# Runki2018/litehandnet

Hardware: AMD Instinct MI355X
Metric: images/sec fwd+bwd @256x256 bs64 litehandnet (higher is better)
Workload: dtype f32; 1 GPU; litehandnet variant B (MSRB hourglass litehourglass.py) C=128, 256x256x3 -> 21x64x64, per-GPU batch 64, train-mode BN, fwd + TopdownHeatmapLoss + bwd + fused Adam; global_batch=64, parallelism=dp1

## Files before the change

### include/lhn.h

```cpp
#ifndef LHN_H
#define LHN_H
#include <stdint.h>
#ifdef __cplusplus
extern "C" {
#endif

#define LHN_VERSION 3
#define LHN_STAT_REPLICAS 32

typedef struct lhn_view {
  float*       data;
  const float* table;
  const float* gate;
  int32_t N, H, W;
  int32_t cstride;
  int32_t coff;
  int32_t C;
  const void* pend;
} lhn_view;

typedef struct lhn_gradview {
  const float* dz;
  const float* dpool;
  const float* coef;
// ... 278 lines not shown
  double*      sums[2];
  int32_t      lo[2], C[2];
  int32_t      n;
} lhn_bn_slices;
int lhn_gate_bwd_reduce2(const lhn_view* y, const float* dz, float* dgate , float* tsum,
                         const lhn_bn_slices* slices, void* stream);
int lhn_gate_bwd_reduce3(const lhn_view* y, const float* dz, float* dgate, float* tsum, const lhn_bn_slices* slices, int prezeroed,
                         void* stream);
typedef struct lhn_gatesum {
  float*               dgate;
  const lhn_bn_slices* slices;
} lhn_gatesum;
int lhn_conv_pw_bwd5(const lhn_view* x, const float* w, const lhn_view* y, const lhn_gradview* gy, float* dx, int dx_accumulate,
                     float* dw, float* dbias, int stride, const float* dy_nchw, int nrep, int64_t rep_stride,
                     const lhn_pw_opts* opts, const lhn_bnsum* bns, const lhn_bnbwdsrc* fin, const lhn_gatesum* gs, void* stream);
int lhn_avgpool_fwd3(const lhn_view* x, float* out , int OH, int OW, float* pstat ,
                     const lhn_bn_slices* slices, void* stream);
int lhn_ca_mlp_bwd2(const float* pooled, const float* w3, const float* gamma, const float* w1, const float* w2,
                    const float* dropmask, const float* save, const float* dgate, float* dpool, int cstride, int coff, int H,
                    int W, float* dw3, float* dgamma, float* dbeta, float* dw1, float* db1, float* dw2, float* db2, int N, int C,
                    int stage, double* gsum, double count_scale, float pgrad_scale, const float* tsum, const float* pstat,
                    const lhn_bn_slices* slices, void* stream);
int lhn_avgpool_fwd4(const lhn_view* x, float* out, int OH, int OW, float* pstat, const lhn_bn_slices* slices,
                     const lhn_view* copy_src, void* stream);
int lhn_ca_mlp_bwd(const float* pooled, const float* w3, const float* gamma, const float* w1, const float* w2,
                   const float* dropmask, const float* save, const float* dgate, float* dpool ,
                   int cstride, int coff, int H, int W, float* dw3, float* dgamma, float* dbeta, float* dw1,
                   float* db1, float* dw2, float* db2, int N, int C, int stage, double* gsum, double count_scale,
                   float pgrad_scale, void* stream);

// ... 14 lines not shown
  int32_t out_buf, out_coff, out_C;
  int32_t p[12];
  int64_t ws[12];
  int32_t i[8];
  float   f[8];
} lhn_op;

typedef struct lhn_buf {
  int64_t data_off, table_off, gate_off, grad_off, dpool_off, coef_off;
  int32_t N, H, W, C;
} lhn_buf;

void* lhn_plan_create(const lhn_buf* bufs, int nbufs, const lhn_op* fwd, int nfwd, const lhn_op* bwd, int nbwd);
void  lhn_plan_destroy(void* plan);
int   lhn_plan_head_gate_fold(void* plan);
#define LHN_RUN_TABLES_CURRENT 2
#define LHN_RUN_GRAPH 4
int   lhn_plan_run(void* plan, int phase, void* workspace, void* const* params, void* const* grads,
                   void* const* io, int training, int grad_replicas, int64_t grad_rep_stride, void* stream);

#ifdef __cplusplus
}
#endif
#endif
```

### litehandnet_amd/_lib.py

```python
import ctypes as C
import os

import torch

_HERE = os.path.dirname(os.path.abspath(__file__))
LIB_PATH = os.path.join(_HERE, "liblhn.so")
_lib = None


class LhnError(RuntimeError):
    pass


class View(C.Structure):
    _fields_ = [("data", C.c_void_p), ("table", C.c_void_p), ("gate", C.c_void_p),
                ("N", C.c_int32), ("H", C.c_int32), ("W", C.c_int32),
                ("cstride", C.c_int32), ("coff", C.c_int32), ("C", C.c_int32), ("pend", C.c_void_p)]


class GradView(C.Structure):
    _fields_ = [("dz", C.c_void_p), ("dpool", C.c_void_p), ("coef", C.c_void_p)]


class Op(C.Structure):
# ... 5 lines not shown

class Buf(C.Structure):
    _fields_ = [("data_off", C.c_int64), ("table_off", C.c_int64), ("gate_off", C.c_int64),
                ("grad_off", C.c_int64), ("dpool_off", C.c_int64), ("coef_off", C.c_int64),
                ("N", C.c_int32), ("H", C.c_int32), ("W", C.c_int32), ("C", C.c_int32)]


SYMBOLS = [
    "lhn_version", "lhn_deterministic", "lhn_last_error", "lhn_device_ok",
    "lhn_heatmap_encode", "lhn_heatmap_argmax", "lhn_heatmap_refine", "lhn_transform_preds",
    "lhn_heatmap_decode", "lhn_heatmap_decode_dark", "lhn_heatmap_decode_dark_udp", "lhn_heatmap_nms", "lhn_heatmap_topk", "lhn_pck_accuracy",
    "lhn_eval_state_bytes", "lhn_eval_accumulate", "lhn_eval_finalize",
    "lhn_loss_balanced_mse_fwd", "lhn_loss_balanced_mse_bwd", "lhn_affine_warp_normalize", "lhn_affine_warp_normalize2", "lhn_random_flip", "lhn_hsv_jitter", "lhn_simdr_encode", "lhn_simdr_loss_fwd", "lhn_simdr_loss_bwd",
    "lhn_conv_pw_fwd", "lhn_conv_pw_fwd2", "lhn_conv_pw_bwd2", "lhn_conv_dw_fwd", "lhn_conv_dw_fwd2", "lhn_conv_dw_fwd3", "lhn_conv_pw_dw3_fwd", "lhn_conv_dw3_pw_fwd", "lhn_msrb_round_scratch_bytes", "lhn_msrb_round_fwd", "lhn_bottleneck_fwd", "lhn_stem_tail_fwd", "lhn_conv_stem_fwd", "lhn_conv_kxk_fwd", "lhn_conv_kxk_fwd_bf16x3",
    "lhn_bn_finalize", "lhn_table_fill", "lhn_table_bias", "lhn_fold_bn", "lhn_ew_fwd", "lhn_ew_fwd2", "lhn_ew_fwd3", "lhn_ew_mul_bwd", "lhn_bilinear_bwd", "lhn_shuffle2_fwd", "lhn_shuffle2_bwd", "lhn_bn_finalize2", "lhn_bn_bwd_finalize2", "lhn_maxpool2_fwd", "lhn_avgpool_fwd", "lhn_avgpool_fwd2", "lhn_avgpool_bwd2", "lhn_se_mlp_fwd2", "lhn_se_mlp_bwd2", "lhn_ca_mlp_fwd", "lhn_att_mlp_fwd", "lhn_att_mlp_bwd", "lhn_se_mlp_fwd", "lhn_se_mlp_bwd",
    "lhn_bn_bwd_reduce", "lhn_bn_bwd_finalize", "lhn_conv_pw_bwd", "lhn_conv_dw_bwd", "lhn_conv_dw_bwd2", "lhn_conv_dw_bwd3", "lhn_conv_dw_bwd4", "lhn_conv_pw_bwd4", "lhn_conv_pw_bwd5", "lhn_plan_head_gate_fold", "lhn_conv_stem_bwd",
    "lhn_conv_kxk_bwd", "lhn_ew_bwd", "lhn_ew_bwd2", "lhn_maxpool2_bwd", "lhn_maxpool2_bwd2", "lhn_maxpool2_bwd3", "lhn_ew_bwd3", "lhn_ew_bwd_multi", "lhn_avgpool_bwd3", "lhn_conv_pw_bwd3", "lhn_avgpool_bwd", "lhn_gate_bwd_reduce", "lhn_gate_bwd_reduce2", "lhn_gate_bwd_reduce3", "lhn_adam_step", "lhn_avgpool_fwd3", "lhn_avgpool_fwd4", "lhn_ca_mlp_bwd2",
    "lhn_ca_mlp_bwd", "lhn_reduce_replicas", "lhn_fold_stat_replicas", "lhn_plan_create", "lhn_plan_destroy", "lhn_plan_run", "lhn_plan_run_range",
    "lhn_cbam_layout", "lhn_cbam_fwd", "lhn_cbam_bwd",
]


def lib():
    global _lib
    if _lib is None:
        if not os.path.exists(LIB_PATH):
            raise LhnError(f"{LIB_PATH} is missing: run `python -m litehandnet_amd.build` "
                           "(hipcc --offload-arch=gfx950); there is no CPU fallback")
        _lib = C.CDLL(LIB_PATH)
        _lib.lhn_last_error.restype = C.c_char_p
        _lib.lhn_plan_create.restype = C.c_void_p
# ... 56 lines not shown
```

### litehandnet_amd/csrc/k_conv_dw.hip

```cpp
#include <stdlib.h>
#include "lhn_common.h"

template <int K>
__global__ void __launch_bounds__(256) k_dw_fwd(lhn_view x, const float* __restrict__ w, lhn_view y,
                                                double* __restrict__ stats, int stride, int pad, int dil, lhn_bnfin fin,
                                                int ) {
  extern __shared__ __attribute__((aligned(16))) float smem[];
  const int C = x.C, C4 = C >> 2;
  constexpr int KK = K * K;
  float* Ws = smem;
  f4* red = reinterpret_cast<f4*>(smem + KK * C);
  const int tid = threadIdx.x;
  const int c4 = tid % C4, pl = tid / C4, PL = 256 / C4;
  const int cin = x.coff + 4 * c4, cout = y.coff + 4 * c4;
  const Xf4 xf = lhn_load_xf(x, cin);
  for (int i = tid; i < KK * C; i += 256) {
    const int c = i / KK, t = i - c * KK;
    Ws[t * C + c] = w ? w[i] : 1.f;
  }
  __syncthreads();
  f4 wt[KK];
#pragma unroll
  for (int t = 0; t < KK; ++t) wt[t] = *reinterpret_cast<const f4*>(Ws + t * C + 4 * c4);
  const int rows = y.N * y.H;
// ... 1178 lines not shown
  if (stats) {
    const int C = x.C;
    double* st = stats + (size_t)((bid / cgroups) % LHN_STAT_REPLICAS) * 2 * C + cg * 32;
    lhn_block_stat_atomics_d(sd, qd, 8, reinterpret_cast<double*>(red), st, st + C, cvalid);
    if (fin.counter && lhn_last_block(fin.counter)) lhn_bn_finalize_block_par(fin, stats, reinterpret_cast<double*>(red));
  }
}

struct DwBnSum {
  double* sums;
  const float* save;
  int C, coff;
  const float* add[2];
};

template <int K, int DIL, bool BNS = false>
__global__ void __launch_bounds__(256) k_dwk_bwd_lds(lhn_view x, const float* __restrict__ w, lhn_view y, lhn_gradview gy,
                                                     float* __restrict__ dx, int dx_acc, float* __restrict__ dw, int tiles_h,
                                                     int tiles_w, int cgroups, int nrep, int64_t rep_stride, int ps, DwBnSum bs, int xchunk) {
  constexpr int TH = 8, TW = 16, KK = K * K;
  const int bid = xchunk ? (int)(blockIdx.x & 7) * xchunk + (int)(blockIdx.x >> 3) : (int)blockIdx.x;
  constexpr bool REGACC = (K == 3);
  using T = DwTile<K, DIL, TH, TW>;
  extern __shared__ __attribute__((aligned(16))) float smem[];
  f4* tdy = reinterpret_cast<f4*>(smem);
  f4* tx = tdy + T::PIX * 8;
  f4* red = tx + T::PIX * 8;
  f4* wl = red + 256;
  f4* dws = wl + KK * 8;
  f4* traw = dws + KK * 8;
  f4* tmi = traw + TH * TW * 8;
  const int tid = threadIdx.x, c4 = tid & 7, pl = tid >> 3;
  const int colw = pl & 15, rpar = pl >> 4;
  const int ntile = y.N * ps * ps * tiles_h * tiles_w * cgroups;
  const int cg = bid % cgroups;
  const int cvalid = min(8, (x.C - cg * 32) >> 2);
  const bool cok = c4 < cvalid;
  const int c4e = cok ? c4 : 0;
  const int cx = x.coff + cg * 32 + 4 * c4e, cy = y.coff + cg * 32 + 4 * c4e;
  const Xf4 xxf = lhn_load_xf(x, cx), yxf = lhn_load_xf(y, cy);
  const Gr4 ygr = lhn_load_coef(gy, y.cstride, cy);
  for (int i = tid; i < KK * 8; i += 256) {
    const int k = i >> 3, cc = cg * 32 + 4 * min(i & 7, cvalid - 1);
    wl[i] = (f4){w[(cc + 0) * KK + k], w[(cc + 1) * KK + k], w[(cc + 2) * KK + k], w[(cc + 3) * KK + k]};
    if (!REGACC) dws[i] = (f4){0.f, 0.f, 0.f, 0.f};
  }
  f4 accw[REGACC ? KK : 1];
#pragma unroll
  for (int k = 0; k < (REGACC ? KK : 1); ++k) accw[k] = (f4){0.f, 0.f, 0.f, 0.f};
  f4 sdu = (f4){0.f, 0.f, 0.f, 0.f}, sdux = sdu;
  if (BNS && tid < 16) {
    const int kind = tid >> 3, cc = tid & 7;
    tmi[tid] = *reinterpret_cast<const f4*>(bs.save + kind * bs.C + bs.coff + cg * 32 + 4 * cc);
  }
  for (int t = bid; t < ntile; t += gridDim.x) {
    int r = t / cgroups;
// ... 395 lines not shown
static void launch_dwk_fwd(const lhn_view* x, const float* w, const lhn_view* y, double* stats, lhn_bnfin fin, hipStream_t s, int ps = 1,
                           const DwExtra* exp = nullptr) {
  DwExtra ex;
  if (exp) ex = *exp; else { ex.n = 0; ex.sum_out = nullptr; }
  constexpr int TH = 8, TW = 32, P = DIL * (K - 1) / 2;
  const int cg = (x->C + 31) / 32;
  const int sh = (y->H + ps - 1) / ps, sw = (y->W + ps - 1) / ps;
  const int th = (sh + TH - 1) / TH, tw = (sw + TW - 1) / TW, ntile = y->N * ps * ps * th * tw * cg;
  const size_t lds = (size_t)((TH + 2 * P) * (TW + 2 * P) * 8 + 512 + K * K * 8) * 16;
  const int per_cu = lds > 80 * 1024 ? 1 : (lds > 52 * 1024 ? 2 : 3);
  static LhnKernelCfg cfg;
  (void)lhn_kernel_cfg(cfg, &k_dwk_fwd_lds<K, DIL, NS>, lds, 4, nullptr);
  const int grid = dw3_grid(ntile, cg, per_cu * 2);
  hipLaunchKernelGGL((k_dwk_fwd_lds<K, DIL, NS>), dim3(grid), dim3(256), lds, s, *x, w, *y, stats, th, tw, cg, fin, ps, ex, dw3_xchunk(grid, cg));
}
template <int K, int DIL, bool BNS = false>
static void launch_dwk_bwd(const lhn_view* x, const float* w, const lhn_view* y, const lhn_gradview* gy, float* dx, int dx_acc,
                           float* dw, int nrep, int64_t rep_stride, hipStream_t s, int ps = 1, const DwBnSum* bsp = nullptr) {
  constexpr int TH = 8, TW = 16, P = DIL * (K - 1) / 2;
  DwBnSum bs;
  if (bsp) bs = *bsp; else { bs.sums = nullptr; bs.save = nullptr; bs.C = bs.coff = 0; bs.add[0] = bs.add[1] = nullptr; }
  const int cg = (x->C + 31) / 32;
  const int sh = (x->H + ps - 1) / ps, sw = (x->W + ps - 1) / ps;
  const int th = (sh + TH - 1) / TH, tw = (sw + TW - 1) / TW, ntile = x->N * ps * ps * th * tw * cg;
  const size_t lds = (size_t)((TH + 2 * P) * (TW + 2 * P) * 16 + 256 + 2 * K * K * 8 + (BNS ? TH * TW * 8 + 16 : 0)) * 16;
  static LhnKernelCfg cfg;
  (void)lhn_kernel_cfg(cfg, &k_dwk_bwd_lds<K, DIL, BNS>, lds, 4, nullptr);
  const int grid = dw3_grid(ntile, cg, 4);
  hipLaunchKernelGGL((k_dwk_bwd_lds<K, DIL, BNS>), dim3(grid), dim3(256), lds, s, *x, w, *y, *gy, dx, dx_acc, dw, th, tw,
                     cg, nrep, rep_stride, ps, bs, dw3_xchunk(grid, cg));
}
template <int DIL, bool BNS = false>
static void launch_dw3_bwd_rows(const lhn_view* x, const float* w, const lhn_view* y, const lhn_gradview* gy, float* dx, int dx_acc,
                                float* dw, int nrep, int64_t rep_stride, hipStream_t s, int ps = 1, const DwBnSum* bsp = nullptr,
                                const lhn_bnbwdsrc* fsp = nullptr) {
  constexpr int P = DIL, R = 2 * P + 2, WW = 32 + 2 * P;
  DwBnSum bs;
  if (bsp) bs = *bsp; else { bs.sums = nullptr; bs.save = nullptr; bs.C = bs.coff = 0; bs.add[0] = bs.add[1] = nullptr; }
  lhn_bnbwdsrc fs;
  if (fsp) fs = *fsp; else memset(&fs, 0, sizeof(fs));
  static_assert(R * WW * 8 * 16 >= 2 * LHN_FIN_THREADS * 8, "dy ring holds the replica fold's partials");
  const int cg = (x->C + 31) / 32;
  const int sh = (x->H + ps - 1) / ps, sw = (x->W + ps - 1) / ps;
  const int nstrips = (sw + 31) / 32;
  const size_t lds = (size_t)(2 * R * WW * 8 + 2 * 9 * 8 + 16 + (BNS ? R * 32 * 8 : 0)) * 16;
// ... 6 lines not shown
  const int CH = (sh + nch - 1) / nch;
  nch = (sh + CH - 1) / CH;
  const int ntile = base * nch;
  const int grid = dw3_grid(ntile, cg, per_cu);
  hipLaunchKernelGGL((k_dw3_bwd_rows<DIL, BNS>), dim3(grid), dim3(256), lds, s, *x, w, *y, *gy, dx, dx_acc, dw, nstrips, nch, CH, cg,
                     nrep, rep_stride, ps, bs, fs);
}
static bool lhn_dw_bwd_v1() {
  static int v = -1;
  if (v < 0) {
    const char* e = getenv("LHN_DW_BWD_V1");
    v = (e && e[0] == '1') ? 1 : 0;
  }
  return v == 1;
}


struct DwS2 {
  static constexpr int TH = 4, TW = 16, XH = 2 * TH + 1, XW = 2 * TW + 1, XPIX = XH * XW, DH = TH + 1, DW = TW + 1, DPIX = DH * DW;
};

__global__ void __launch_bounds__(256) k_dws2_fwd_lds(lhn_view x, const float* __restrict__ w, lhn_view y, double* __restrict__ stats,
                                                      int tiles_h, int tiles_w, int cgroups, lhn_bnfin fin) {
  using T = DwS2;
  extern __shared__ __attribute__((aligned(16))) float smem[];
  f4* tx = reinterpret_cast<f4*>(smem);
  f4* red = tx + T::XPIX * 8;
  f4* wl = red + 512;
  const int tid = threadIdx.x, c4 = tid & 7, pl = tid >> 3;
  const int ntile = y.N * tiles_h * tiles_w * cgroups;
// ... 237 lines not shown
    else if (k == 3 && dil == 2 && y->W >= 16) launch_dwk_fwd<3, 1, 2>(x, w, y, stats, fin, s, 2, ex);
    else return 0;
    return 1;
  }
  if (k == 3 && dil == 1) launch_dwk_fwd<3, 1>(x, w, y, stats, fin, s, 1, ex);
  else if (k == 3 && dil == 2 && y->W >= 16) launch_dwk_fwd<3, 1>(x, w, y, stats, fin, s, 2, ex);
  else if (k == 3 && dil == 2) launch_dwk_fwd<3, 2>(x, w, y, stats, fin, s, 1, ex);
  else if (k == 7 && dil == 1) launch_dwk_fwd<7, 1>(x, w, y, stats, fin, s, 1, ex);
  else return 0;
  return 1;
}
int lhn_dwk_bwd_lds(const lhn_view* x, const float* w, const lhn_view* y, const lhn_gradview* gy, float* dx, int dx_acc,
                    float* dw, int k, int dil, int nrep, int64_t rep_stride, hipStream_t s, const DwBnSum* bs,
                    const lhn_bnbwdsrc* fs) {
  if (fs && (lhn_dw_bwd_v1() || k != 3)) return 0;
  if (bs && bs->sums) {
    if (!(k == 3 && dil == 1 && dx && !dx_acc)) return 0;
    if (lhn_dw_bwd_v1()) launch_dwk_bwd<3, 1, true>(x, w, y, gy, dx, dx_acc, dw, nrep, rep_stride, s, 1, bs);
    else launch_dw3_bwd_rows<1, true>(x, w, y, gy, dx, dx_acc, dw, nrep, rep_stride, s, 1, bs, fs);
    return 1;
  }
  const bool v1 = lhn_dw_bwd_v1();
  if (k == 3 && dil == 1) {
    if (v1) launch_dwk_bwd<3, 1>(x, w, y, gy, dx, dx_acc, dw, nrep, rep_stride, s, 1, bs);
    else launch_dw3_bwd_rows<1>(x, w, y, gy, dx, dx_acc, dw, nrep, rep_stride, s, 1, bs, fs);
  } else if (k == 3 && dil == 2 && x->W >= 16) {
    if (v1) launch_dwk_bwd<3, 1>(x, w, y, gy, dx, dx_acc, dw, nrep, rep_stride, s, 2, bs);
    else launch_dw3_bwd_rows<1>(x, w, y, gy, dx, dx_acc, dw, nrep, rep_stride, s, 2, bs, fs);
  } else if (k == 3 && dil == 2) {
    if (v1) launch_dwk_bwd<3, 2>(x, w, y, gy, dx, dx_acc, dw, nrep, rep_stride, s, 1, bs);
    else launch_dw3_bwd_rows<2>(x, w, y, gy, dx, dx_acc, dw, nrep, rep_stride, s, 1, bs, fs);
  } else if (k == 7 && dil == 1) launch_dwk_bwd<7, 1>(x, w, y, gy, dx, dx_acc, dw, nrep, rep_stride, s, 1, bs);
  else return 0;
  return 1;
}

static int dw_fwd_extra(const lhn_view* x, const float* w, const lhn_view* y, double* stats, int k, int stride, int pad, int dil,
                        lhn_bnfin fin, const lhn_view* extra, const float* coef, const lhn_view* so, hipStream_t s) {
  if (!(stride == 1 && pad == dil * (k - 1) / 2 && x->C % 4 == 0 && y->W >= 8)) return 0;
// ... 47 lines not shown
```

### litehandnet_amd/csrc/k_conv_pw.hip

```cpp
#include <stdlib.h>
#include "lhn_common.h"

struct PwGeom {
  int wstride, kvalid, wrows, yacc, statC;
  int64_t nchw_bstride;
};

template <int CIN>
__device__ __forceinline__ void pw_stage_w(float* Ws, int LDA, const float* __restrict__ w, int rows_pad, const PwGeom& g) {
  constexpr int C4 = CIN / 4;
  const bool vec = (g.wstride % 4 == 0) && (g.kvalid % 4 == 0) && ((reinterpret_cast<uintptr_t>(w) & 15) == 0);
  for (int i = threadIdx.x; i < rows_pad * C4; i += 256) {
    const int co = i / C4, k4 = i % C4;
    f4 v = (f4){0.f, 0.f, 0.f, 0.f};
    if (co < g.wrows) {
      const float* r = w + (int64_t)co * g.wstride + k4 * 4;
      if (vec) {
        if (4 * k4 < g.kvalid) v = *reinterpret_cast<const f4*>(r);
      } else {
        if (4 * k4 + 0 < g.kvalid) v.x = r[0];
        if (4 * k4 + 1 < g.kvalid) v.y = r[1];
        if (4 * k4 + 2 < g.kvalid) v.z = r[2];
        if (4 * k4 + 3 < g.kvalid) v.w = r[3];
      }
// ... 1242 lines not shown
                                int64_t rep_stride, const lhn_pw_opts* opts, void* stream) {
  return lhn_conv_pw_bwd3(x, w, y, gy, dx, dx_accumulate, dw, dbias, stride, dy_nchw, nrep, rep_stride, opts, nullptr, stream);
}
extern "C" int lhn_conv_pw_bwd3(const lhn_view* x, const float* w, const lhn_view* y, const lhn_gradview* gy, float* dx,
                                int dx_accumulate, float* dw, float* dbias, int stride, const float* dy_nchw, int nrep,
                                int64_t rep_stride, const lhn_pw_opts* opts, const lhn_bnsum* bns, void* stream) {
  return lhn_conv_pw_bwd4(x, w, y, gy, dx, dx_accumulate, dw, dbias, stride, dy_nchw, nrep, rep_stride, opts, bns, nullptr, stream);
}
extern "C" int lhn_conv_pw_bwd4(const lhn_view* x, const float* w, const lhn_view* y, const lhn_gradview* gy, float* dx,
                                int dx_accumulate, float* dw, float* dbias, int stride, const float* dy_nchw, int nrep,
                                int64_t rep_stride, const lhn_pw_opts* opts, const lhn_bnsum* bns, const lhn_bnbwdsrc* fin, void* stream) {
  return lhn_conv_pw_bwd5(x, w, y, gy, dx, dx_accumulate, dw, dbias, stride, dy_nchw, nrep, rep_stride, opts, bns, fin, nullptr, stream);
}
static int pw_bwd_run(const lhn_view* x, const float* w, const lhn_view* y, const lhn_gradview* gy, float* dx, int dx_accumulate, float* dw,
                      float* dbias, int stride, const float* dy_nchw, int nrep, int64_t rep_stride, const lhn_pw_opts* opts,
                      const lhn_bnsum* bns, const lhn_bnbwdsrc* fin, const lhn_gatesum* gs, bool* gs_done, void* stream);
extern "C" int lhn_conv_pw_bwd5(const lhn_view* x, const float* w, const lhn_view* y, const lhn_gradview* gy, float* dx,
                                int dx_accumulate, float* dw, float* dbias, int stride, const float* dy_nchw, int nrep,
                                int64_t rep_stride, const lhn_pw_opts* opts, const lhn_bnsum* bns, const lhn_bnbwdsrc* fin,
                                const lhn_gatesum* gs, void* stream) {
  if (gs && !gs->dgate) gs = nullptr;
  if (gs) LHN_CHECK_ARG(lhn_view_ok(x) && dx && !dx_accumulate && stride == 1 && (!gs->slices || (gs->slices->n >= 0 && gs->slices->n <= 2)),
                        "lhn_conv_pw_bwd5: gate sums need a stored dx (no accumulate), stride 1 and 0..2 BatchNorm slices");
  bool gs_done = false;
  const int rc = pw_bwd_run(x, w, y, gy, dx, dx_accumulate, dw, dbias, stride, dy_nchw, nrep, rep_stride, opts, bns, fin, gs, &gs_done, stream);
  if (rc || !gs || gs_done) return rc;
  lhn_view xv = *x;
  xv.gate = nullptr;
  return lhn_gate_bwd_reduce3(&xv, dx, gs->dgate, gs->dgate + (size_t)x->N * x->cstride, gs->slices, 1, stream);
}
static int pw_bwd_run(const lhn_view* x, const float* w, const lhn_view* y, const lhn_gradview* gy, float* dx, int dx_accumulate, float* dw,
                      float* dbias, int stride, const float* dy_nchw, int nrep, int64_t rep_stride, const lhn_pw_opts* opts,
                      const lhn_bnsum* bns, const lhn_bnbwdsrc* fin, const lhn_gatesum* gs, bool* gs_done, void* stream) {
  if (nrep < 1) nrep = 1;
  if (fin && !fin->sums) fin = nullptr;
  lhn_bnsum bs;
  memset(&bs, 0, sizeof(bs));
  if (bns && bns->sums) {
    LHN_CHECK_ARG(x && y && bns->save && dx && stride == 1 && x->C <= 128 && y->C <= 128 && x->C * y->C < 64 * 128 && !x->gate && x->table &&
                      bns->coff >= 0 && bns->coff + x->C <= bns->C,
                  "lhn_conv_pw_bwd3: BatchNorm sums ride in the fused kernel only (stride 1, Cin * Cout < 8192, ungated input inside the producer's channels)");
    bs = *bns;
  }
  LHN_CHECK_ARG(lhn_view_ok(x) && w && y && gy && dw && lhn_no_pend(x) && lhn_no_pend(y), "lhn_conv_pw_bwd: bad view / null pointer");
  LHN_CHECK_ARG(stride == 1 || stride == 2, "lhn_conv_pw_bwd: stride %d", stride);
  LHN_CHECK_ARG(stride == 1 || !dx || dx_accumulate, "lhn_conv_pw_bwd: stride-2 dgrad only accumulates into a zeroed gradient");
  if (!dy_nchw) LHN_CHECK_ARG(lhn_view_ok(y) && gy->dz, "lhn_conv_pw_bwd: bad output view / missing dz");
  const int Cout = y->C, Cin = x->C, HoWo = y->H * y->W;
// ... 15 lines not shown
    *gs_done = gs != nullptr;
    return 0;
  }
  if (fin) {
    LHN_CHECK_ARG(!dy_nchw && gy->coef && fin->save_mean_invstd && fin->count > 0 && fin->stat_channels >= Cout,
                  "lhn_conv_pw_bwd4: finalize source needs gy->coef, saved statistics and stat_channels >= Cout");
    if (!wr_wide && !wr_narrow) {
      const int rc = lhn_bn_bwd_finalize2(fin->sums, fin->gamma, fin->save_mean_invstd, const_cast<float*>(gy->coef), y->cstride, y->coff,
                                          Cout, fin->stat_channels, fin->count, fin->dgamma, fin->dbeta, fin->pgrad_scale, stream);
      if (rc) return rc;
      fin = nullptr;
    }
  }
  if (wr_wide) {
    int rc = -1;
    if (Cin == 128 && Cout == 128) rc = launch_pw_bwd_wr<128, 128, 32, 1>(x, w, y, gy, dx, dx_accumulate, dw, dbias, nrep, rep_stride, s, bs, fin);
    else if (Cin == 64 && Cout == 128) rc = launch_pw_bwd_wr<64, 128, 64, 1>(x, w, y, gy, dx, dx_accumulate, dw, dbias, nrep, rep_stride, s, bs, fin);
    else if (Cin == 128 && Cout == 64) rc = launch_pw_bwd_wr<128, 64, 64, 2>(x, w, y, gy, dx, dx_accumulate, dw, dbias, nrep, rep_stride, s, bs, fin);
    if (rc == 0) {
      LHN_CHECK_LAUNCH("lhn_conv_pw_bwd");
      return 0;
    }
    if (rc > 0) return rc;
  }
  if (wr_narrow) {
    int rc;
    if (Cin == 64) rc = bs.sums ? launch_pw_bwd_wr<64, 64, 64, 2, false, true>(x, w, y, gy, dx, dx_accumulate, dw, dbias, nrep, rep_stride, s, bs, fin)
                                : launch_pw_bwd_wr<64, 64, 64, 2, false, false>(x, w, y, gy, dx, dx_accumulate, dw, dbias, nrep, rep_stride, s, bs, fin);
    else rc = bs.sums ? launch_pw_bwd_wr<32, 32, 128, 2, false, true>(x, w, y, gy, dx, dx_accumulate, dw, dbias, nrep, rep_stride, s, bs, fin)
                      : launch_pw_bwd_wr<32, 32, 128, 2, false, false, 3>(x, w, y, gy, dx, dx_accumulate, dw, dbias, nrep, rep_stride, s, bs, fin);
    if (rc) return rc;
    LHN_CHECK_LAUNCH("lhn_conv_pw_bwd");
    return 0;
// ... 52 lines not shown
```

### litehandnet_amd/csrc/lhn_plan.cpp

```cpp
#include <stdint.h>
#include <stdlib.h>
#include <string.h>
#include <vector>
#include "lhn_common.h"

static lhn_bnsum mkbns(void* ws, int64_t sums_off, int64_t save_off, int C, int coff) {
  lhn_bnsum b;
  memset(&b, 0, sizeof(b));
  if (sums_off >= 0 && save_off >= 0 && C > 0) {
    b.sums = reinterpret_cast<double*>(static_cast<char*>(ws) + sums_off);
    b.save = reinterpret_cast<const float*>(static_cast<char*>(ws) + save_off);
    b.C = C;
    b.coff = coff;
  }
  return b;
}

enum {
  OP_STEM = 1, OP_PW = 2, OP_DW = 3, OP_KXK = 4, OP_FINALIZE = 5, OP_EW = 6, OP_MAXPOOL = 7, OP_AVGPOOL = 8,
  OP_CA_MLP = 9, OP_TABLE_FILL = 10, OP_MEMSET = 11, OP_ATT_MLP = 12, OP_SE_MLP = 13, OP_SHUFFLE = 14,
  OP_PWDW = 15, OP_DWPW = 16, OP_MSRB = 17, OP_CBAM = 18, OP_BNECK = 19, OP_STEMTAIL = 20,
  OP_STEM_BWD = 101, OP_PW_BWD = 102, OP_DW_BWD = 103, OP_KXK_BWD = 104, OP_BN_BWD = 105, OP_EW_BWD = 106,
  OP_MAXPOOL_BWD = 107, OP_AVGPOOL_BWD = 108, OP_GATE_REDUCE = 109, OP_CA_MLP_BWD = 110, OP_ATT_MLP_BWD = 111, OP_SE_MLP_BWD = 112,
  OP_SHUFFLE_BWD = 113, OP_CBAM_BWD = 114,
};

struct GraphEntry {
  int phase, training, nrep, seen;
  int64_t rstr;
  void *ws, *io0, *io1;
  uint64_t phash, ghash;
  hipGraphExec_t exec;
  uint64_t last_use;
};

struct Plan {
  std::vector<lhn_buf> bufs;
  std::vector<lhn_op> fwd, bwd;
  std::vector<GraphEntry> graphs;
  uint64_t tick = 0;
  int graph_misses = 0;
};

static inline char* at(void* ws, int64_t off) { return off < 0 ? nullptr : static_cast<char*>(ws) + off; }

static lhn_view mkview(const Plan* P, void* ws, int buf, int coff, int C, bool with_gate = true) {
  const lhn_buf& b = P->bufs[buf];
  lhn_view v;
  v.pend = nullptr;
  v.data = reinterpret_cast<float*>(at(ws, b.data_off));
  v.table = reinterpret_cast<const float*>(at(ws, b.table_off));
  v.gate = with_gate ? reinterpret_cast<const float*>(at(ws, b.gate_off)) : nullptr;
  v.N = b.N; v.H = b.H; v.W = b.W;
// ... 56 lines not shown
    const char* e = getenv("LHN_BWD_FIN_CONSUMER");
    v = (e && e[0] == '0') ? 0 : 1;
  }
  return v == 1;
}
bool lhn_head_stream_on();
static bool head_gate_fold_at(const Plan* P, const std::vector<lhn_op>& ops, size_t oi) {
  if (!lhn_head_stream_on() || lhn_deterministic_mode() || oi + 1 >= ops.size()) return false;
  const lhn_op &o = ops[oi], &nx = ops[oi + 1];
  if (o.kind != OP_PW_BWD || !o.i[1] || o.i[0] != 1 || o.i[2] != 1 || o.in_buf[0] < 0) return false;
  if (o.in_C[0] != 128 || o.out_C > 32 || o.i[3] || o.i[4]) return false;
  const lhn_buf& b = P->bufs[o.in_buf[0]];
  return o.in_coff[0] == 0 && o.in_C[0] == b.C && b.gate_off >= 0 && nx.kind == OP_GATE_REDUCE && nx.out_buf == o.in_buf[0] &&
         nx.out_coff == 0 && nx.out_C == b.C && nx.ws[3] >= 0 && nx.ws[4] >= 0;
}

static int sep_finalize(const lhn_bnfin& f, const double* stats, int training, void* stream, int creal = 0, int repeat = 1) {
  int rc = 0;
  for (int r = 0; r < (training ? (repeat < 1 ? 1 : repeat) : 1) && !rc; ++r)
    rc = lhn_bn_finalize2(training ? stats : nullptr, f.gamma, f.beta, f.running_mean, f.running_var,
                          training ? f.num_batches_tracked : nullptr, f.table, f.cstride, f.coff, creal > 0 ? creal : f.C, f.C,
                          training ? f.save_mean_invstd : nullptr, f.count, f.eps, f.momentum, f.slope, training, f.conv_bias, stream);
  return rc;
}

extern "C" {

void* lhn_plan_create(const lhn_buf* bufs, int nbufs, const lhn_op* fwd, int nfwd, const lhn_op* bwd, int nbwd) {
  if (!bufs || nbufs <= 0 || !fwd || nfwd <= 0) {
    lhn_set_error("lhn_plan_create: empty plan");
// ... 1 lines not shown
  }
  Plan* p = new Plan();
  p->bufs.assign(bufs, bufs + nbufs);
  p->fwd.assign(fwd, fwd + nfwd);
  if (bwd && nbwd > 0) p->bwd.assign(bwd, bwd + nbwd);
  for (const auto* lst : {&p->fwd, &p->bwd})
    for (const lhn_op& o : *lst) {
      bool ok = o.out_buf < nbufs;
      for (int k = 0; k < 3; ++k) ok = ok && o.in_buf[k] < nbufs;
      if (!ok) {
        lhn_set_error("lhn_plan_create: op kind %d references buffer out of range", o.kind);
        delete p;
        return nullptr;
      }
    }
  return p;
}

int lhn_plan_head_gate_fold(void* plan) {
  const Plan* p = static_cast<const Plan*>(plan);
  if (!p) return -1;
  for (size_t oi = 0; oi + 1 < p->bwd.size(); ++oi)
    if (head_gate_fold_at(p, p->bwd, oi)) return (int)oi + 1;
  return -1;
}

void lhn_plan_destroy(void* plan) {
  Plan* p = static_cast<Plan*>(plan);
  if (!p) return;
  for (GraphEntry& g : p->graphs)
    if (g.exec) (void)hipGraphExecDestroy(g.exec);
  delete p;
}

static int run_ops(const Plan* P, int phase, void* ws, void* const* params, void* const* grads, void* const* io, int mode,
                   int nrep, int64_t rstr, void* stream, size_t sb = 0, size_t se = (size_t)-1, double cscale = 1.0,
                   float pscale = 1.f) {
  const int training = mode & 1;
  const bool skip_tables = (mode & 2) != 0 && !training;
// ... 348 lines not shown
          const int64_t khw = (int64_t)o.out_C * y.H * y.W;
          nchw += (int64_t)o.i[6] * khw;
          po.nchw_batch_stride = (int64_t)o.i[7] * khw;
        }
        const lhn_bnsum bs = mkbns(ws, o.ws[0], o.ws[1], (int)o.f[6], (int)o.f[7]);
        lhn_gatesum gsum;
        lhn_bn_slices gsl;
        memset(&gsum, 0, sizeof(gsum));
        if (phase == 1 && whole && head_gate_fold_at(P, ops, oi)) {
          const lhn_op& nx = ops[oi + 1];
          gsl = mkslices(ws, &nx.i[0], &nx.ws[5], nullptr);
          gsum.dgate = reinterpret_cast<float*>(at(ws, nx.ws[3]));
          gsum.slices = &gsl;
          gfold_at = oi + 1;
        }
        rc = lhn_conv_pw_bwd5(&x, prm<const float>(params, o.p[0]), &y, &g, dx, o.i[2] == 2, prm<float>(grads, o.p[1]),
                              prm<float>(grads, o.p[2]), o.i[0], nchw, nrep, rstr, &po, bs.sums ? &bs : nullptr,
                              cfin_for == oi ? &cfin : nullptr, gsum.dgate ? &gsum : nullptr, stream);
        break;
      }
      case OP_DW_BWD: {
        lhn_view x = mkview(P, ws, o.in_buf[0], o.in_coff[0], o.in_C[0]);
        lhn_view y = mkview(P, ws, o.out_buf, o.out_coff, o.out_C);
        lhn_gradview g = mkgrad(P, ws, o.out_buf, o.i[5] != 0);
        float* dx = o.i[4] ? reinterpret_cast<float*>(at(ws, P->bufs[o.in_buf[0]].grad_off)) : nullptr;
        if (cfin_for == oi) {
          const bool adds = o.ws[2] >= 0 || o.ws[3] >= 0;
          const lhn_bnsum bs = mkbns(ws, adds ? -1 : o.ws[4], adds ? -1 : o.ws[5], o.i[6], o.i[7]);
          rc = lhn_conv_dw_bwd4(&x, prm<const float>(params, o.p[0]), &y, &g, dx, o.i[4] == 2, prm<float>(grads, o.p[1]), o.i[0], o.i[1],
                                o.i[2], o.i[3], nrep, rstr, bs.sums ? &bs : nullptr,
                                o.ws[2] >= 0 ? reinterpret_cast<const float*>(at(ws, o.ws[2])) : nullptr,
                                o.ws[3] >= 0 ? reinterpret_cast<const float*>(at(ws, o.ws[3])) : nullptr, &cfin, stream);
          break;
// ... 304 lines not shown
```

Measured before the change: 9268 images/s.

## Skip dead dy stores in pointwise bwd and fold BN coef into small dw bwd

Adds a plan-time liveness analysis that marks pointwise-conv backward ops whose output gradient buffer is never read again, and passes a flag so the wide backward kernel skips writing back the transformed dy. It also routes small-spatial 3x3 depthwise backward to the LDS tile kernel with an in-kernel BN backward coefficient fold instead of the row kernel. The intent is to cut redundant global writes and a separate coefficient pass. The risk is that the liveness check misses an alias and drops a needed store, and that the LDS kernel is slower than the row kernel on some shapes.

```diff
diff --git a/include/lhn.h b/include/lhn.h
--- a/include/lhn.h
+++ b/include/lhn.h
@@ -316,6 +316,11 @@
 int lhn_conv_pw_bwd5(const lhn_view* x, const float* w, const lhn_view* y, const lhn_gradview* gy, float* dx, int dx_accumulate,
                      float* dw, float* dbias, int stride, const float* dy_nchw, int nrep, int64_t rep_stride,
                      const lhn_pw_opts* opts, const lhn_bnsum* bns, const lhn_bnbwdsrc* fin, const lhn_gatesum* gs, void* stream);
+#define LHN_PW_BWD_DZ_DEAD 1
+int lhn_conv_pw_bwd6(const lhn_view* x, const float* w, const lhn_view* y, const lhn_gradview* gy, float* dx, int dx_accumulate,
+                     float* dw, float* dbias, int stride, const float* dy_nchw, int nrep, int64_t rep_stride,
+                     const lhn_pw_opts* opts, const lhn_bnsum* bns, const lhn_bnbwdsrc* fin, const lhn_gatesum* gs, int flags,
+                     void* stream);
 int lhn_avgpool_fwd3(const lhn_view* x, float* out , int OH, int OW, float* pstat ,
                      const lhn_bn_slices* slices, void* stream);
 int lhn_ca_mlp_bwd2(const float* pooled, const float* w3, const float* gamma, const float* w1, const float* w2,
@@ -360,6 +365,7 @@
 void* lhn_plan_create(const lhn_buf* bufs, int nbufs, const lhn_op* fwd, int nfwd, const lhn_op* bwd, int nbwd);
 void  lhn_plan_destroy(void* plan);
 int   lhn_plan_head_gate_fold(void* plan);
+int   lhn_plan_pw_dz_dead(void* plan, int bwd_index);
 #define LHN_RUN_TABLES_CURRENT 2
 #define LHN_RUN_GRAPH 4
 int   lhn_plan_run(void* plan, int phase, void* workspace, void* const* params, void* const* grads,
diff --git a/litehandnet_amd/_lib.py b/litehandnet_amd/_lib.py
--- a/litehandnet_amd/_lib.py
+++ b/litehandnet_amd/_lib.py
@@ -43,7 +43,7 @@
     "lhn_loss_balanced_mse_fwd", "lhn_loss_balanced_mse_bwd", "lhn_affine_warp_normalize", "lhn_affine_warp_normalize2", "lhn_random_flip", "lhn_hsv_jitter", "lhn_simdr_encode", "lhn_simdr_loss_fwd", "lhn_simdr_loss_bwd",
     "lhn_conv_pw_fwd", "lhn_conv_pw_fwd2", "lhn_conv_pw_bwd2", "lhn_conv_dw_fwd", "lhn_conv_dw_fwd2", "lhn_conv_dw_fwd3", "lhn_conv_pw_dw3_fwd", "lhn_conv_dw3_pw_fwd", "lhn_msrb_round_scratch_bytes", "lhn_msrb_round_fwd", "lhn_bottleneck_fwd", "lhn_stem_tail_fwd", "lhn_conv_stem_fwd", "lhn_conv_kxk_fwd", "lhn_conv_kxk_fwd_bf16x3",
     "lhn_bn_finalize", "lhn_table_fill", "lhn_table_bias", "lhn_fold_bn", "lhn_ew_fwd", "lhn_ew_fwd2", "lhn_ew_fwd3", "lhn_ew_mul_bwd", "lhn_bilinear_bwd", "lhn_shuffle2_fwd", "lhn_shuffle2_bwd", "lhn_bn_finalize2", "lhn_bn_bwd_finalize2", "lhn_maxpool2_fwd", "lhn_avgpool_fwd", "lhn_avgpool_fwd2", "lhn_avgpool_bwd2", "lhn_se_mlp_fwd2", "lhn_se_mlp_bwd2", "lhn_ca_mlp_fwd", "lhn_att_mlp_fwd", "lhn_att_mlp_bwd", "lhn_se_mlp_fwd", "lhn_se_mlp_bwd",
-    "lhn_bn_bwd_reduce", "lhn_bn_bwd_finalize", "lhn_conv_pw_bwd", "lhn_conv_dw_bwd", "lhn_conv_dw_bwd2", "lhn_conv_dw_bwd3", "lhn_conv_dw_bwd4", "lhn_conv_pw_bwd4", "lhn_conv_pw_bwd5", "lhn_plan_head_gate_fold", "lhn_conv_stem_bwd",
+    "lhn_bn_bwd_reduce", "lhn_bn_bwd_finalize", "lhn_conv_pw_bwd", "lhn_conv_dw_bwd", "lhn_conv_dw_bwd2", "lhn_conv_dw_bwd3", "lhn_conv_dw_bwd4", "lhn_conv_pw_bwd4", "lhn_conv_pw_bwd5", "lhn_conv_pw_bwd6", "lhn_plan_head_gate_fold", "lhn_plan_pw_dz_dead", "lhn_conv_stem_bwd",
     "lhn_conv_kxk_bwd", "lhn_ew_bwd", "lhn_ew_bwd2", "lhn_maxpool2_bwd", "lhn_maxpool2_bwd2", "lhn_maxpool2_bwd3", "lhn_ew_bwd3", "lhn_ew_bwd_multi", "lhn_avgpool_bwd3", "lhn_conv_pw_bwd3", "lhn_avgpool_bwd", "lhn_gate_bwd_reduce", "lhn_gate_bwd_reduce2", "lhn_gate_bwd_reduce3", "lhn_adam_step", "lhn_avgpool_fwd3", "lhn_avgpool_fwd4", "lhn_ca_mlp_bwd2",
     "lhn_ca_mlp_bwd", "lhn_reduce_replicas", "lhn_fold_stat_replicas", "lhn_plan_create", "lhn_plan_destroy", "lhn_plan_run", "lhn_plan_run_range",
     "lhn_cbam_layout", "lhn_cbam_fwd", "lhn_cbam_bwd",
diff --git a/litehandnet_amd/csrc/k_conv_dw.hip b/litehandnet_amd/csrc/k_conv_dw.hip
--- a/litehandnet_amd/csrc/k_conv_dw.hip
+++ b/litehandnet_amd/csrc/k_conv_dw.hip
@@ -1216,10 +1216,11 @@
   const float* add[2];
 };
 
-template <int K, int DIL, bool BNS = false>
+template <int K, int DIL, bool BNS = false, bool FOLD = false>
 __global__ void __launch_bounds__(256) k_dwk_bwd_lds(lhn_view x, const float* __restrict__ w, lhn_view y, lhn_gradview gy,
                                                      float* __restrict__ dx, int dx_acc, float* __restrict__ dw, int tiles_h,
-                                                     int tiles_w, int cgroups, int nrep, int64_t rep_stride, int ps, DwBnSum bs, int xchunk) {
+                                                     int tiles_w, int cgroups, int nrep, int64_t rep_stride, int ps, DwBnSum bs, int xchunk,
+                                                     lhn_bnbwdsrc fs) {
   constexpr int TH = 8, TW = 16, KK = K * K;
   const int bid = xchunk ? (int)(blockIdx.x & 7) * xchunk + (int)(blockIdx.x >> 3) : (int)blockIdx.x;
   constexpr bool REGACC = (K == 3);
@@ -1232,6 +1233,7 @@
   f4* dws = wl + KK * 8;
   f4* traw = dws + KK * 8;
   f4* tmi = traw + TH * TW * 8;
+  float* cfA = reinterpret_cast<float*>(BNS ? tmi + 16 : traw);
   const int tid = threadIdx.x, c4 = tid & 7, pl = tid >> 3;
   const int colw = pl & 15, rpar = pl >> 4;
   const int ntile = y.N * ps * ps * tiles_h * tiles_w * cgroups;
@@ -1241,7 +1243,24 @@
   const int c4e = cok ? c4 : 0;
   const int cx = x.coff + cg * 32 + 4 * c4e, cy = y.coff + cg * 32 + 4 * c4e;
   const Xf4 xxf = lhn_load_xf(x, cx), yxf = lhn_load_xf(y, cy);
-  const Gr4 ygr = lhn_load_coef(gy, y.cstride, cy);
+  Gr4 ygr;
+  if (FOLD && fs.sums) {
+    static_assert(!FOLD || T::PIX * 8 * sizeof(f4) >= 2 * LHN_FIN_THREADS * sizeof(double), "dy tile holds the replica fold's partials");
+    double* raw = reinterpret_cast<double*>(tdy);
+    const int nc = 4 * cvalid;
+    const LhnBwdPre pre = lhn_bn_bwd_pre(fs, cg * 32, nc);
+    lhn_bn_bwd_fold_raw(fs.sums, fs.stat_channels, cg * 32, nc, raw);
+    __syncthreads();
+    if (tid < nc)
+      lhn_bn_bwd_coef_put(lhn_bn_bwd_coef_raw(raw, nc, lhn_fin_groups(y.C), tid, pre, fs.count), fs, const_cast<float*>(gy.coef), y.cstride,
+                          y.coff, cg * 32 + tid, cfA, 32, tid, bid < cgroups);
+    __syncthreads();
+    ygr.A = *reinterpret_cast<const f4*>(cfA + 4 * c4e);
+    ygr.B = *reinterpret_cast<const f4*>(cfA + 32 + 4 * c4e);
+    ygr.Cc = *reinterpret_cast<const f4*>(cfA + 64 + 4 * c4e);
+  } else {
+    ygr = lhn_load_coef(gy, y.cstride, cy);
+  }
   for (int i = tid; i < KK * 8; i += 256) {
     const int k = i >> 3, cc = cg * 32 + 4 * min(i & 7, cvalid - 1);
     wl[i] = (f4){w[(cc + 0) * KK + k], w[(cc + 1) * KK + k], w[(cc + 2) * KK + k], w[(cc + 3) * KK + k]};
@@ -1667,21 +1686,24 @@
   const int grid = dw3_grid(ntile, cg, per_cu * 2);
   hipLaunchKernelGGL((k_dwk_fwd_lds<K, DIL, NS>), dim3(grid), dim3(256), lds, s, *x, w, *y, stats, th, tw, cg, fin, ps, ex, dw3_xchunk(grid, cg));
 }
-template <int K, int DIL, bool BNS = false>
+template <int K, int DIL, bool BNS = false, bool FOLD = false>
 static void launch_dwk_bwd(const lhn_view* x, const float* w, const lhn_view* y, const lhn_gradview* gy, float* dx, int dx_acc,
-                           float* dw, int nrep, int64_t rep_stride, hipStream_t s, int ps = 1, const DwBnSum* bsp = nullptr) {
+                           float* dw, int nrep, int64_t rep_stride, hipStream_t s, int ps = 1, const DwBnSum* bsp = nullptr,
+                           const lhn_bnbwdsrc* fsp = nullptr) {
   constexpr int TH = 8, TW = 16, P = DIL * (K - 1) / 2;
   DwBnSum bs;
   if (bsp) bs = *bsp; else { bs.sums = nullptr; bs.save = nullptr; bs.C = bs.coff = 0; bs.add[0] = bs.add[1] = nullptr; }
+  lhn_bnbwdsrc fs;
+  if (FOLD && fsp) fs = *fsp; else memset(&fs, 0, sizeof(fs));
   const int cg = (x->C + 31) / 32;
   const int sh = (x->H + ps - 1) / ps, sw = (x->W + ps - 1) / ps;
   const int th = (sh + TH - 1) / TH, tw = (sw + TW - 1) / TW, ntile = x->N * ps * ps * th * tw * cg;
-  const size_t lds = (size_t)((TH + 2 * P) * (TW + 2 * P) * 16 + 256 + 2 * K * K * 8 + (BNS ? TH * TW * 8 + 16 : 0)) * 16;
+  const size_t lds = (size_t)((TH + 2 * P) * (TW + 2 * P) * 16 + 256 + 2 * K * K * 8 + (BNS ? TH * TW * 8 + 16 : 0) + (FOLD ? 24 : 0)) * 16;
   static LhnKernelCfg cfg;
-  (void)lhn_kernel_cfg(cfg, &k_dwk_bwd_lds<K, DIL, BNS>, lds, 4, nullptr);
+  (void)lhn_kernel_cfg(cfg, &k_dwk_bwd_lds<K, DIL, BNS, FOLD>, lds, 4, nullptr);
   const int grid = dw3_grid(ntile, cg, 4);
-  hipLaunchKernelGGL((k_dwk_bwd_lds<K, DIL, BNS>), dim3(grid), dim3(256), lds, s, *x, w, *y, *gy, dx, dx_acc, dw, th, tw,
-                     cg, nrep, rep_stride, ps, bs, dw3_xchunk(grid, cg));
+  hipLaunchKernelGGL((k_dwk_bwd_lds<K, DIL, BNS, FOLD>), dim3(grid), dim3(256), lds, s, *x, w, *y, *gy, dx, dx_acc, dw, th, tw,
+                     cg, nrep, rep_stride, ps, bs, dw3_xchunk(grid, cg), fs);
 }
 template <int DIL, bool BNS = false>
 static void launch_dw3_bwd_rows(const lhn_view* x, const float* w, const lhn_view* y, const lhn_gradview* gy, float* dx, int dx_acc,
@@ -1718,6 +1740,14 @@
   }
   return v == 1;
 }
+static bool dw_bwd_small(const lhn_view* x) {
+  static int v = -1;
+  if (v < 0) {
+    const char* e = getenv("LHN_DW_BWD_SMALL");
+    v = (e && e[0] == '0') ? 0 : 1;
+  }
+  return v == 1 && (int64_t)x->H * x->W <= 256;
+}
 
 
 struct DwS2 {
@@ -1985,15 +2015,18 @@
                     float* dw, int k, int dil, int nrep, int64_t rep_stride, hipStream_t s, const DwBnSum* bs,
                     const lhn_bnbwdsrc* fs) {
   if (fs && (lhn_dw_bwd_v1() || k != 3)) return 0;
+  const bool small = k == 3 && dil == 1 && dw_bwd_small(x);
   if (bs && bs->sums) {
     if (!(k == 3 && dil == 1 && dx && !dx_acc)) return 0;
     if (lhn_dw_bwd_v1()) launch_dwk_bwd<3, 1, true>(x, w, y, gy, dx, dx_acc, dw, nrep, rep_stride, s, 1, bs);
+    else if (small) launch_dwk_bwd<3, 1, true, true>(x, w, y, gy, dx, dx_acc, dw, nrep, rep_stride, s, 1, bs, fs);
     else launch_dw3_bwd_rows<1, true>(x, w, y, gy, dx, dx_acc, dw, nrep, rep_stride, s, 1, bs, fs);
     return 1;
   }
   const bool v1 = lhn_dw_bwd_v1();
   if (k == 3 && dil == 1) {
     if (v1) launch_dwk_bwd<3, 1>(x, w, y, gy, dx, dx_acc, dw, nrep, rep_stride, s, 1, bs);
+    else if (small) launch_dwk_bwd<3, 1, false, true>(x, w, y, gy, dx, dx_acc, dw, nrep, rep_stride, s, 1, bs, fs);
     else launch_dw3_bwd_rows<1>(x, w, y, gy, dx, dx_acc, dw, nrep, rep_stride, s, 1, bs, fs);
   } else if (k == 3 && dil == 2 && x->W >= 16) {
     if (v1) launch_dwk_bwd<3, 1>(x, w, y, gy, dx, dx_acc, dw, nrep, rep_stride, s, 2, bs);
diff --git a/litehandnet_amd/csrc/k_conv_pw.hip b/litehandnet_amd/csrc/k_conv_pw.hip
--- a/litehandnet_amd/csrc/k_conv_pw.hip
+++ b/litehandnet_amd/csrc/k_conv_pw.hip
@@ -1280,16 +1280,22 @@
 }
 static int pw_bwd_run(const lhn_view* x, const float* w, const lhn_view* y, const lhn_gradview* gy, float* dx, int dx_accumulate, float* dw,
                       float* dbias, int stride, const float* dy_nchw, int nrep, int64_t rep_stride, const lhn_pw_opts* opts,
-                      const lhn_bnsum* bns, const lhn_bnbwdsrc* fin, const lhn_gatesum* gs, bool* gs_done, void* stream);
+                      const lhn_bnsum* bns, const lhn_bnbwdsrc* fin, const lhn_gatesum* gs, bool* gs_done, int flags, void* stream);
 extern "C" int lhn_conv_pw_bwd5(const lhn_view* x, const float* w, const lhn_view* y, const lhn_gradview* gy, float* dx,
                                 int dx_accumulate, float* dw, float* dbias, int stride, const float* dy_nchw, int nrep,
                                 int64_t rep_stride, const lhn_pw_opts* opts, const lhn_bnsum* bns, const lhn_bnbwdsrc* fin,
                                 const lhn_gatesum* gs, void* stream) {
+  return lhn_conv_pw_bwd6(x, w, y, gy, dx, dx_accumulate, dw, dbias, stride, dy_nchw, nrep, rep_stride, opts, bns, fin, gs, 0, stream);
+}
+extern "C" int lhn_conv_pw_bwd6(const lhn_view* x, const float* w, const lhn_view* y, const lhn_gradview* gy, float* dx,
+                                int dx_accumulate, float* dw, float* dbias, int stride, const float* dy_nchw, int nrep,
+                                int64_t rep_stride, const lhn_pw_opts* opts, const lhn_bnsum* bns, const lhn_bnbwdsrc* fin,
+                                const lhn_gatesum* gs, int flags, void* stream) {
   if (gs && !gs->dgate) gs = nullptr;
   if (gs) LHN_CHECK_ARG(lhn_view_ok(x) && dx && !dx_accumulate && stride == 1 && (!gs->slices || (gs->slices->n >= 0 && gs->slices->n <= 2)),
                         "lhn_conv_pw_bwd5: gate sums need a stored dx (no accumulate), stride 1 and 0..2 BatchNorm slices");
   bool gs_done = false;
-  const int rc = pw_bwd_run(x, w, y, gy, dx, dx_accumulate, dw, dbias, stride, dy_nchw, nrep, rep_stride, opts, bns, fin, gs, &gs_done, stream);
+  const int rc = pw_bwd_run(x, w, y, gy, dx, dx_accumulate, dw, dbias, stride, dy_nchw, nrep, rep_stride, opts, bns, fin, gs, &gs_done, flags, stream);
   if (rc || !gs || gs_done) return rc;
   lhn_view xv = *x;
   xv.gate = nullptr;
@@ -1297,7 +1303,7 @@
 }
 static int pw_bwd_run(const lhn_view* x, const float* w, const lhn_view* y, const lhn_gradview* gy, float* dx, int dx_accumulate, float* dw,
                       float* dbias, int stride, const float* dy_nchw, int nrep, int64_t rep_stride, const lhn_pw_opts* opts,
-                      const lhn_bnsum* bns, const lhn_bnbwdsrc* fin, const lhn_gatesum* gs, bool* gs_done, void* stream) {
+                      const lhn_bnsum* bns, const lhn_bnbwdsrc* fin, const lhn_gatesum* gs, bool* gs_done, int flags, void* stream) {
   if (nrep < 1) nrep = 1;
   if (fin && !fin->sums) fin = nullptr;
   lhn_bnsum bs;
@@ -1343,9 +1349,13 @@
   }
   if (wr_wide) {
     int rc = -1;
-    if (Cin == 128 && Cout == 128) rc = launch_pw_bwd_wr<128, 128, 32, 1>(x, w, y, gy, dx, dx_accumulate, dw, dbias, nrep, rep_stride, s, bs, fin);
-    else if (Cin == 64 && Cout == 128) rc = launch_pw_bwd_wr<64, 128, 64, 1>(x, w, y, gy, dx, dx_accumulate, dw, dbias, nrep, rep_stride, s, bs, fin);
-    else if (Cin == 128 && Cout == 64) rc = launch_pw_bwd_wr<128, 64, 64, 2>(x, w, y, gy, dx, dx_accumulate, dw, dbias, nrep, rep_stride, s, bs, fin);
+#define PWB_WIDE(CI, CO, PXV, PFV) \
+  if (Cin == CI && Cout == CO)     \
+    rc = dz_dead ? launch_pw_bwd_wr<CI, CO, PXV, PFV, false>(x, w, y, gy, dx, dx_accumulate, dw, dbias, nrep, rep_stride, s, bs, fin) \
+                 : launch_pw_bwd_wr<CI, CO, PXV, PFV, true>(x, w, y, gy, dx, dx_accumulate, dw, dbias, nrep, rep_stride, s, bs, fin);
+    const bool dz_dead = (flags & LHN_PW_BWD_DZ_DEAD) != 0;
+    PWB_WIDE(128, 128, 32, 1) PWB_WIDE(64, 128, 64, 1) PWB_WIDE(128, 64, 64, 2)
+#undef PWB_WIDE
     if (rc == 0) {
       LHN_CHECK_LAUNCH("lhn_conv_pw_bwd");
       return 0;
diff --git a/litehandnet_amd/csrc/lhn_plan.cpp b/litehandnet_amd/csrc/lhn_plan.cpp
--- a/litehandnet_amd/csrc/lhn_plan.cpp
+++ b/litehandnet_amd/csrc/lhn_plan.cpp
@@ -37,6 +37,7 @@
 struct Plan {
   std::vector<lhn_buf> bufs;
   std::vector<lhn_op> fwd, bwd;
+  std::vector<uint8_t> pw_dz_dead;
   std::vector<GraphEntry> graphs;
   uint64_t tick = 0;
   int graph_misses = 0;
@@ -123,6 +124,45 @@
   return o.in_coff[0] == 0 && o.in_C[0] == b.C && b.gate_off >= 0 && nx.kind == OP_GATE_REDUCE && nx.out_buf == o.in_buf[0] &&
          nx.out_coff == 0 && nx.out_C == b.C && nx.ws[3] >= 0 && nx.ws[4] >= 0;
 }
+static bool pw_bwd_dy_store() {
+  static int v = -1;
+  if (v < 0) {
+    const char* e = getenv("LHN_PW_BWD_DY_STORE");
+    v = (e && e[0] == '1') ? 1 : 0;
+  }
+  return v == 1;
+}
+static bool pw_dz_dead_at(const Plan* P, const std::vector<lhn_op>& ops, size_t oi) {
+  const lhn_op& o = ops[oi];
+  if (o.kind != OP_PW_BWD || o.i[1] || o.out_buf < 0 || P->bufs[o.out_buf].grad_off < 0) return false;
+  auto grad_bytes = [&](int buf, int64_t* lo, int64_t* hi) {
+    const lhn_buf& b = P->bufs[buf];
+    *lo = b.grad_off;
+    *hi = b.grad_off + (int64_t)sizeof(float) * b.N * b.H * b.W * b.C;
+    return b.grad_off >= 0;
+  };
+  int64_t lo, hi;
+  grad_bytes(o.out_buf, &lo, &hi);
+  const int oC = P->bufs[o.out_buf].C;
+  auto touches = [&](int buf, int coff, int C) {
+    int64_t a, b;
+    if (buf < 0 || !grad_bytes(buf, &a, &b) || a >= hi || lo >= b) return false;
+    return a != lo || P->bufs[buf].C != oC || (coff < o.out_coff + o.out_C && o.out_coff < coff + C);
+  };
+  for (size_t k = oi + 1; k < ops.size(); ++k) {
+    const lhn_op& q = ops[k];
+    if (q.kind == OP_MEMSET) {
+      if (q.ws[0] < hi && lo < q.ws[0] + q.ws[1]) return false;
+      continue;
+    }
+    if (touches(q.out_buf, q.out_coff, q.out_C)) return false;
+    for (int s = 0; s < 3; ++s)
+      if (touches(q.in_buf[s], q.in_coff[s], q.in_C[s])) return false;
+    for (int s = 0; s < 12; ++s)
+      if (q.ws[s] >= lo && q.ws[s] < hi) return false;
+  }
+  return true;
+}
 
 static int sep_finalize(const lhn_bnfin& f, const double* stats, int training, void* stream, int creal = 0, int repeat = 1) {
   int rc = 0;
@@ -154,6 +194,8 @@
         return nullptr;
       }
     }
+  p->pw_dz_dead.resize(p->bwd.size());
+  for (size_t oi = 0; oi < p->bwd.size(); ++oi) p->pw_dz_dead[oi] = pw_dz_dead_at(p, p->bwd, oi) ? 1 : 0;
   return p;
 }
 
@@ -163,6 +205,12 @@
   for (size_t oi = 0; oi + 1 < p->bwd.size(); ++oi)
     if (head_gate_fold_at(p, p->bwd, oi)) return (int)oi + 1;
   return -1;
+}
+
+int lhn_plan_pw_dz_dead(void* plan, int bwd_index) {
+  const Plan* p = static_cast<const Plan*>(plan);
+  if (!p || bwd_index < 0 || (size_t)bwd_index >= p->pw_dz_dead.size()) return -1;
+  return p->pw_dz_dead[bwd_index];
 }
 
 void lhn_plan_destroy(void* plan) {
@@ -541,9 +589,10 @@
           gsum.slices = &gsl;
           gfold_at = oi + 1;
         }
-        rc = lhn_conv_pw_bwd5(&x, prm<const float>(params, o.p[0]), &y, &g, dx, o.i[2] == 2, prm<float>(grads, o.p[1]),
+        const int flags = (phase == 1 && whole && P->pw_dz_dead[oi] && !pw_bwd_dy_store()) ? LHN_PW_BWD_DZ_DEAD : 0;
+        rc = lhn_conv_pw_bwd6(&x, prm<const float>(params, o.p[0]), &y, &g, dx, o.i[2] == 2, prm<float>(grads, o.p[1]),
                               prm<float>(grads, o.p[2]), o.i[0], nchw, nrep, rstr, &po, bs.sums ? &bs : nullptr,
-                              cfin_for == oi ? &cfin : nullptr, gsum.dgate ? &gsum : nullptr, stream);
+                              cfin_for == oi ? &cfin : nullptr, gsum.dgate ? &gsum : nullptr, flags, stream);
         break;
       }
       case OP_DW_BWD: {
```

Measured after the change: 9380 images/s (median of 6 runs). +1.2%, better.
